# KochPJ/AutoPoseEstimation

Hardware: AMD Instinct MI355X
Metric: RGB-D frames/sec (seg+DenseFusion+2-refine), 640x480 N=1000 (higher is better)
Workload: dtype bf16x3

## Files before the change

### autoposeestimation_amd/csrc/conv_gemm.hip

```cpp
#include "s32.h"

namespace {

using namespace ape;

struct GemmArgs {
    const float* x;
    const __bf16* w;
    const float* bias;
    const float* res;
    float* y;
    ape_conv_params p;
    int M, Kp, m_tiles, n_tiles, nk;
    int out_fmt;
    int dbg;
    long plane_stride;
    int nk_per;
    long split_stride;
};

constexpr int BK = 32;

template <int NSPLIT, int BM, int BN, int WM, int WN, bool PURE, bool PP, bool SK>
__device__ __forceinline__ void conv_gemm_body(const GemmArgs& a, const int orig)
// ... 276 lines not shown
                }
            }
        }
    }
}

template <int NSPLIT, int BM, int BN, int WM, int WN, bool PURE, bool PP>
__global__ __launch_bounds__(WM * WN * 64, 2) void conv_gemm_kernel(const GemmArgs a)
{
    conv_gemm_body<NSPLIT, BM, BN, WM, WN, PURE, PP, false>(a, (int)blockIdx.x);
}

template <int NSPLIT, bool PURE>
__global__ __launch_bounds__(256, 2) void conv_gemm_splitk_kernel(const GemmArgs a)
{
    conv_gemm_body<NSPLIT, 128, 128, 2, 2, PURE, false, true>(a, (int)blockIdx.x);
}

constexpr int kMultiMax = 4;
struct GemmMultiArgs {
    GemmArgs a[kMultiMax];
    int first[kMultiMax + 1];
};
template <int NSPLIT>
__global__ __launch_bounds__(256, 2) void conv_gemm_multi_kernel(const GemmMultiArgs m)
{
    const int blk = (int)blockIdx.x;
    int pi = 0;
#pragma unroll
    for (int i = 1; i < kMultiMax; ++i) pi = blk >= m.first[i] ? i : pi;
    conv_gemm_body<NSPLIT, 128, 128, 2, 2, true, false, false>(m.a[pi], blk - m.first[pi]);
}

template <int NSPLIT, int BM, int BN, int WM, int WN, bool PP = false>
void launch(GemmArgs& a, bool pure, hipStream_t st)
{
    a.m_tiles = ape::ceil_div(a.M, BM);
    a.n_tiles = ape::ceil_div(a.p.Cout, BN);
    if (pure)
        hipLaunchKernelGGL((conv_gemm_kernel<NSPLIT, BM, BN, WM, WN, true, PP>), dim3(a.m_tiles * a.n_tiles), dim3(WM * WN * 64), 0, st, a);
    else
        hipLaunchKernelGGL((conv_gemm_kernel<NSPLIT, BM, BN, WM, WN, false, PP>), dim3(a.m_tiles * a.n_tiles), dim3(WM * WN * 64), 0, st, a);
}

template <int NSPLIT>
void launch_splitk(GemmArgs& a, bool pure, hipStream_t st)
{
    a.m_tiles = ape::ceil_div(a.M, 128);
    a.n_tiles = ape::ceil_div(a.p.Cout, 128);
    const int gy = ape::ceil_div(a.nk, a.nk_per);
    if (pure)
        hipLaunchKernelGGL((conv_gemm_splitk_kernel<NSPLIT, true>), dim3(a.m_tiles * a.n_tiles, gy), dim3(256), 0, st, a);
    else
        hipLaunchKernelGGL((conv_gemm_splitk_kernel<NSPLIT, false>), dim3(a.m_tiles * a.n_tiles, gy), dim3(256), 0, st, a);
}

__global__ void splitk_finish_kernel(const float* __restrict__ ws, int splits, long M, int Cout, const float* __restrict__ bias, int bias_bstride,
                                     int HoWo, const float* __restrict__ res, int ldr, int roff, float* __restrict__ y, int ldy, int yoff, int act,
                                     float alpha)
{
    const long n = M * Cout;
    for (long i = blockIdx.x * (long)blockDim.x + threadIdx.x; i < n; i += (long)gridDim.x * blockDim.x) {
        const long m = i / Cout;
        const int c = (int)(i - m * Cout);
        float v = ws[i];
        for (int k = 1; k < splits; ++k) v += ws[(long)k * n + i];
// ... 17 lines not shown

bool supported(const ape_conv_params& p)
{
    if (p.B < 0 || p.H < 1 || p.W < 1 || p.Cin < 32 || p.Cin % 32 || p.Cout < 1 || p.KH < 1 || p.KW < 1 || p.stride < 1 ||
        p.dil < 1 || p.pad < 0 || p.Ho < 1 || p.Wo < 1 || p.ups != 0)
        return false;
    if (p.ldx % 4 || p.xoff % 4 || p.xoff + p.Cin > p.ldx || p.yoff + p.Cout > p.ldy) return false;
    if (p.act < APE_ACT_NONE || p.act > APE_ACT_SIGMOID) return false;
    const int ho = (p.H + 2 * p.pad - p.dil * (p.KH - 1) - 1) / p.stride + 1;
    const int wo = (p.W + 2 * p.pad - p.dil * (p.KW - 1) - 1) / p.stride + 1;
    if (ho != p.Ho || wo != p.Wo) return false;
    const long M = (long)p.B * p.Ho * p.Wo;
    if (M > (1L << 30) || (long)p.B * p.H * p.W * p.ldx >= (1L << 31) || (long)p.Cout * p.KH * p.KW * p.Cin >= (1L << 31)) return false;
    return true;
}

}

extern "C" int ape_conv_gemm_supported(const ape_conv_params* params) { return params && supported(*params) ? 1 : 0; }

extern "C" int ape_conv_gemm_bf16(const float* x, const void* w_packed, const float* bias, const float* residual, float* y,
                                  const ape_conv_params* params, int nsplit, int variant, void* stream)
{
    return ape_conv_gemm_bf16_fmt(x, w_packed, bias, residual, y, APE_FMT_F32, params, nsplit, variant, stream);
}

extern "C" int ape_conv_gemm_bf16_fmt(const float* x, const void* w_packed, const float* bias, const float* residual, void* y_, int out_fmt,
                                      const ape_conv_params* params, int nsplit, int variant, void* stream)
{
    float* y = (float*)y_;
    if (out_fmt != APE_FMT_F32 && out_fmt != APE_FMT_S32) return APE_EINVAL;
    if (out_fmt == APE_FMT_S32 && params && (params->ldy % 32 || params->Cout % 4 || params->yoff % 4 || (residual && (params->ldr % 4 || params->roff % 4))))
        return APE_EINVAL;
    if (!x || !w_packed || !y || !params || (nsplit != 1 && nsplit != 3) || variant < 0 || (variant & 15) > 6) return APE_EINVAL;
    const ape_conv_params& p = *params;
    if (!supported(p)) return APE_EINVAL;
    if (residual && p.roff + p.Cout > p.ldr) return APE_EINVAL;
    const long M = (long)p.B * p.Ho * p.Wo;
    if (M == 0) return APE_OK;
    GemmArgs a;
    a.x = x; a.w = (const __bf16*)w_packed; a.bias = bias; a.res = residual; a.y = y; a.p = p;
    a.M = (int)M;
    const int K = p.KH * p.KW * p.Cin;
    a.Kp = (K + 7) / 8 * 8;
    a.nk = K / BK;
    a.plane_stride = (long)p.Cout * a.Kp;
    a.dbg = variant >> 4;
    a.out_fmt = out_fmt;
    a.nk_per = 0;
    a.split_stride = 0;
    variant &= 15;
    const bool pure = p.KH == 1 && p.KW == 1 && p.stride == 1 && p.pad == 0;
    hipStream_t st = (hipStream_t)stream;
    if (variant == 0) {
        const int waste256 = ape::ceil_div(p.Cout, 256) * 256 - p.Cout;
        const int waste192 = ape::ceil_div(p.Cout, 192) * 192 - p.Cout;
        if (p.Cout <= 64) variant = 3;
        else if (p.Cout >= 256 && waste256 * 8 <= p.Cout && K >= 256 && (long)ape::ceil_div(M, 256) * ape::ceil_div(p.Cout, 256) >= 192) variant = 1;
        else if (p.Cout >= 192 && waste192 * 8 <= p.Cout && K >= 256 && (long)ape::ceil_div(M, 256) * ape::ceil_div(p.Cout, 192) >= 192) variant = 4;
        else variant = 2;
    }
    if (variant == 1) {
        if (nsplit == 3) launch<3, 256, 256, 2, 4>(a, pure, st); else launch<1, 256, 256, 2, 4>(a, pure, st);
    } else if (variant == 2) {
        if (nsplit == 3) launch<3, 128, 128, 2, 2>(a, pure, st); else launch<1, 128, 128, 2, 2>(a, pure, st);
    } else if (variant == 3) {
        if (nsplit == 3) launch<3, 256, 64, 4, 1>(a, pure, st); else launch<1, 256, 64, 4, 1>(a, pure, st);
    } else if (variant == 4) {
        if (nsplit == 3) launch<3, 256, 192, 2, 4>(a, pure, st); else launch<1, 256, 192, 2, 4>(a, pure, st);
    } else if (variant == 5) {
        if (nsplit == 3) launch<3, 256, 256, 2, 4, true>(a, pure, st); else launch<1, 256, 256, 2, 4, true>(a, pure, st);
    } else {
        if (nsplit == 3) launch<3, 128, 192, 2, 2>(a, pure, st); else launch<1, 128, 192, 2, 2>(a, pure, st);
    }
    return ape::check_launch("ape_conv_gemm_bf16");
}

extern "C" int ape_conv_gemm_bf16_multi(int n, const float* const* x, const void* const* w_packed, const float* const* bias, float* const* y,
                                        const ape_conv_params* params, int nsplit, void* stream)
{
    if (n < 1 || n > kMultiMax || !x || !w_packed || !y || !params || (nsplit != 1 && nsplit != 3)) return APE_EINVAL;
    GemmMultiArgs m;
    int total = 0;
    for (int i = 0; i < kMultiMax; ++i) {
        m.first[i] = total;
        if (i >= n) { m.a[i] = m.a[0]; continue; }
        const ape_conv_params& p = params[i];
        if (!x[i] || !w_packed[i] || !y[i] || !supported(p) || p.KH != 1 || p.KW != 1 || p.stride != 1 || p.pad != 0) return APE_EINVAL;
        const long M = (long)p.B * p.Ho * p.Wo;
        GemmArgs& a = m.a[i];
        a.x = x[i]; a.w = (const __bf16*)w_packed[i]; a.bias = bias ? bias[i] : nullptr; a.res = nullptr; a.y = y[i]; a.p = p;
        a.M = (int)M;
        a.Kp = (p.Cin + 7) / 8 * 8;
        a.nk = p.Cin / BK;
        a.plane_stride = (long)p.Cout * a.Kp;
        a.dbg = 0;
        a.out_fmt = APE_FMT_F32;
        a.nk_per = 0;
        a.split_stride = 0;
        a.m_tiles = ape::ceil_div(a.M, 128);
        a.n_tiles = ape::ceil_div(p.Cout, 128);
        total += a.m_tiles * a.n_tiles;
// ... 54 lines not shown
```

### autoposeestimation_amd/csrc/ops.hip

```cpp
#include <map>
#include <mutex>
#include "s32.h"

namespace {

using ape::src_index;
constexpr int kThreads = 256;
constexpr int kGridCap = 8192;

__global__ void maxpool3x3s2_kernel(const float4* __restrict__ x, float4* __restrict__ y, int B, int H, int W, int C4,
                                    int Ho, int Wo)
{
    const long total = (long)B * Ho * Wo * C4;
    for (long i = blockIdx.x * (long)blockDim.x + threadIdx.x; i < total; i += (long)gridDim.x * blockDim.x) {
        const int c = i % C4;
        long t = i / C4;
        const int ox = t % Wo; t /= Wo;
        const int oy = t % Ho;
        const int b = t / Ho;
        float4 m = make_float4(-__builtin_inff(), -__builtin_inff(), -__builtin_inff(), -__builtin_inff());
#pragma unroll
        for (int ky = 0; ky < 3; ++ky) {
            const int iy = oy * 2 - 1 + ky;
            if ((unsigned)iy >= (unsigned)H) continue;
// ... 63 lines not shown
            const long row = (long)(b * H + y) * W;
#pragma unroll
            for (int a = 0; a < kPoolMaxAtoms; ++a) {
                if (a >= pl.nx) break;
                int xx = pl.xe[a];
                const int xend = pl.xe[a + 1];
                for (; xx + 4 <= xend; xx += 4) {
                    const float4 v0 = load(row + xx), v1 = load(row + xx + 1), v2 = load(row + xx + 2), v3 = load(row + xx + 3);
                    acc[a].x += v0.x; acc[a].y += v0.y; acc[a].z += v0.z; acc[a].w += v0.w;
                    acc[a].x += v1.x; acc[a].y += v1.y; acc[a].z += v1.z; acc[a].w += v1.w;
                    acc[a].x += v2.x; acc[a].y += v2.y; acc[a].z += v2.z; acc[a].w += v2.w;
                    acc[a].x += v3.x; acc[a].y += v3.y; acc[a].z += v3.z; acc[a].w += v3.w;
                }
                for (; xx < xend; ++xx) {
                    const float4 v = load(row + xx);
                    acc[a].x += v.x; acc[a].y += v.y; acc[a].z += v.z; acc[a].w += v.w;
                }
            }
        }
    }
    if (g > 0) {
#pragma unroll
        for (int a = 0; a < kPoolMaxAtoms; ++a) part[g - 1][a][lane] = acc[a];
    }
    __syncthreads();
    if (g == 0 && c < C4) {
#pragma unroll
        for (int a = 0; a < kPoolMaxAtoms; ++a) {
            if (a >= pl.nx) break;
            float4 t = acc[a];
            for (int k = 0; k < 3; ++k) { t.x += part[k][a][lane].x; t.y += part[k][a][lane].y; t.z += part[k][a][lane].z; t.w += part[k][a][lane].w; }
            atoms[(((long)b * pl.ny + ay) * pl.nx + a) * C4 + c] = t;
        }
    }
}

__global__ void avgpool_bins_kernel(const float4* __restrict__ atoms, const PoolPlan pl, int B, int H, int W, int C4, int bins_total)
{
    const long total = (long)B * bins_total * C4;
    for (long i = blockIdx.x * (long)blockDim.x + threadIdx.x; i < total; i += (long)gridDim.x * blockDim.x) {
        const int c = i % C4;
        long t = i / C4;
        int bin = t % bins_total;
        const int b = t / bins_total;
        int si = 0;
        while (bin >= pl.S[si] * pl.S[si]) { bin -= pl.S[si] * pl.S[si]; ++si; }
        const int S = pl.S[si], oy = bin / S, ox = bin - oy * S;
        float4 acc = make_float4(0.f, 0.f, 0.f, 0.f);
        for (int ay = pl.ya[si][oy]; ay < pl.yb[si][oy]; ++ay)
            for (int ax = pl.xa[si][ox]; ax < pl.xb[si][ox]; ++ax) {
                const float4 v = atoms[(((long)b * pl.ny + ay) * pl.nx + ax) * C4 + c];
                acc.x += v.x; acc.y += v.y; acc.z += v.z; acc.w += v.w;
            }
        const float inv = 1.f / (float)((pl.ye[pl.yb[si][oy]] - pl.ye[pl.ya[si][oy]]) * (pl.xe[pl.xb[si][ox]] - pl.xe[pl.xa[si][ox]]));
        reinterpret_cast<float4*>(pl.out[si])[((long)(b * S + oy) * S + ox) * C4 + c] = make_float4(acc.x * inv, acc.y * inv, acc.z * inv, acc.w * inv);
    }
}

__global__ void bilinear_kernel(const float* __restrict__ x, float* __restrict__ y, int B, int H, int W, int C4, int ldx4,
                                int Ho, int Wo, int ldy4, int yoff4, float sh, float sw, int align_corners, int accumulate)
{
    const float4* x4 = reinterpret_cast<const float4*>(x);
    float4* y4 = reinterpret_cast<float4*>(y);
    const long total = (long)B * Ho * Wo * C4;
    for (long i = blockIdx.x * (long)blockDim.x + threadIdx.x; i < total; i += (long)gridDim.x * blockDim.x) {
        const int c = i % C4;
// ... 541 lines not shown
            cuts[n++] = (o * L) / sizes[i];
            cuts[n++] = ((o + 1) * L + sizes[i] - 1) / sizes[i];
        }
    for (int i = 1; i < n; ++i)
        for (int j = i; j > 0 && cuts[j - 1] > cuts[j]; --j) { const int t = cuts[j]; cuts[j] = cuts[j - 1]; cuts[j - 1] = t; }
    int m = 0;
    for (int i = 0; i < n; ++i)
        if (m == 0 || cuts[i] != edges[m - 1]) {
            if (m > kPoolMaxAtoms) return -1;
            edges[m++] = cuts[i];
        }
    const int atoms = m - 1;
    if (atoms < 1 || atoms > kPoolMaxAtoms) return -1;
    for (int i = 0; i < nsizes; ++i)
        for (int o = 0; o < sizes[i]; ++o) {
            const int lo = (o * L) / sizes[i], hi = ((o + 1) * L + sizes[i] - 1) / sizes[i];
            int a0 = 0, a1 = 0;
            while (edges[a0] != lo) ++a0;
            while (edges[a1] != hi) ++a1;
            first[i][o] = a0;
            end[i][o] = a1;
        }
    return atoms;
}

extern "C" size_t ape_adaptive_avgpool_multi_workspace_bytes(int B, int C)
{
    return (size_t)(B < 0 ? 0 : B) * kPoolMaxAtoms * kPoolMaxAtoms * (size_t)(C < 0 ? 0 : C) * sizeof(float);
}

extern "C" int ape_adaptive_avgpool_multi_nhwc_ld(const void* x, int in_fmt, float* const* ys_host, const int* sizes_host, int nsizes, int B, int H,
                                                  int W, int C, int ldx, void* workspace, size_t workspace_bytes, void* stream)
{
    if ((in_fmt != APE_FMT_F32 && in_fmt != APE_FMT_S32) || (in_fmt == APE_FMT_S32 && (C % 32 || ldx % 32))) return APE_EINVAL;
    if (!x || !ys_host || !sizes_host || !workspace || nsizes < 1 || nsizes > kPoolMaxSizes || B < 0 || H < 1 || W < 1 || C < 4 || C % 4 ||
        ldx < C || ldx % 4)
        return APE_EINVAL;
    if (B == 0) return APE_OK;
    PoolPlan pl;
    pl.nsizes = nsizes;
    int bins_total = 0;
    for (int i = 0; i < nsizes; ++i) {
        if (sizes_host[i] < 1 || sizes_host[i] > kPoolMaxS || !ys_host[i]) return APE_EINVAL;
        pl.S[i] = sizes_host[i];
        pl.out[i] = ys_host[i];
        bins_total += sizes_host[i] * sizes_host[i];
    }
    for (int i = nsizes; i < kPoolMaxSizes; ++i) { pl.S[i] = 1 << 20; pl.out[i] = nullptr; }
    pl.ny = pool_axis_plan(H, sizes_host, nsizes, pl.ye, pl.ya, pl.yb);
    pl.nx = pool_axis_plan(W, sizes_host, nsizes, pl.xe, pl.xa, pl.xb);
    if (pl.ny < 0 || pl.nx < 0) return APE_EINVAL;
    if (workspace_bytes < (size_t)B * pl.ny * pl.nx * C * sizeof(float)) return APE_EWORKSPACE;
    hipStream_t st = (hipStream_t)stream;
    if (in_fmt == APE_FMT_S32)
        hipLaunchKernelGGL(avgpool_atoms_kernel<true>, dim3(B * pl.ny, ape::ceil_div(C / 4, 64)), dim3(256), 0, st, (const float4*)x,
                           (float4*)workspace, pl, H, W, C / 4, ldx / 4);
    else
        hipLaunchKernelGGL(avgpool_atoms_kernel<false>, dim3(B * pl.ny, ape::ceil_div(C / 4, 64)), dim3(256), 0, st, (const float4*)x,
                           (float4*)workspace, pl, H, W, C / 4, ldx / 4);
    const long total = (long)B * bins_total * (C / 4);
    hipLaunchKernelGGL(avgpool_bins_kernel, dim3(ape::grid_for(total, kThreads, kGridCap)), dim3(kThreads), 0, st, (const float4*)workspace, pl, B, H, W, C / 4,
                       bins_total);
    return ape::check_launch("ape_adaptive_avgpool_multi_nhwc_f32");
}

extern "C" int ape_bilinear_nhwc_f32(const float* x, float* y, int B, int H, int W, int C, int ldx, int Ho, int Wo, int ldy,
                                     int yoff, int align_corners, int accumulate, void* stream)
{
    if (!x || !y || B < 0 || H < 1 || W < 1 || Ho < 1 || Wo < 1 || C < 4 || C % 4 || ldx % 4 || ldy % 4 || yoff % 4 ||
        C > ldx || yoff + C > ldy)
        return APE_EINVAL;
    float sh, sw;
    if (align_corners) {
        sh = Ho > 1 ? (float)(H - 1) / (float)(Ho - 1) : 0.f;
        sw = Wo > 1 ? (float)(W - 1) / (float)(Wo - 1) : 0.f;
    } else {
        sh = (float)H / (float)Ho;
        sw = (float)W / (float)Wo;
    }
    const long total = (long)B * Ho * Wo * (C / 4);
    if (total == 0) return APE_OK;
    hipLaunchKernelGGL(bilinear_kernel, dim3(ape::grid_for(total, kThreads, kGridCap)), dim3(kThreads), 0, (hipStream_t)stream, x, y, B, H, W, C / 4,
                       ldx / 4, Ho, Wo, ldy / 4, yoff / 4, sh, sw, align_corners, accumulate);
    return ape::check_launch("ape_bilinear_nhwc_f32");
}

extern "C" int ape_gather_rows_f32(const float* x, const int64_t* index, float* y, int B, int rows_in, int n, int C, void* stream)
{
    if (!x || !index || !y || B < 0 || rows_in < 1 || n < 0 || C < 4 || C % 4) return APE_EINVAL;
    const long total = (long)B * n * (C / 4);
    if (total == 0) return APE_OK;
    hipLaunchKernelGGL(gather_rows_kernel, dim3(ape::grid_for(total, kThreads, kGridCap)), dim3(kThreads), 0, (hipStream_t)stream, (const float4*)x,
// ... 133 lines not shown
```

### autoposeestimation_amd/engine.py

```python
import contextlib
import contextvars
import ctypes
import os

import torch

from . import _lib
from ._lib import ACT_NONE, ACT_PRELU, ACT_RELU, ACT_SIGMOID, ConvParams


def _st():
    return _lib.stream_ptr()


class LaunchProfile:

    def __init__(self, only=None):
        self.records = []
        self.only = only

    def wants(self, label):
        return self.only is None or label in self.only

    def begin(self, label):
# ... 13 lines not shown
        for name, shape, flop, nbytes, e0, e1 in self.records:
            key = (name, shape) if by_shape else name
            d = out.setdefault(key, {"launches": 0, "flop": 0.0, "bytes": 0.0, "ms": 0.0})
            d["launches"] += 1
            d["flop"] += flop
            d["bytes"] += nbytes
            d["ms"] += e0.elapsed_time(e1)
        return out


def _prof_begin(label):
    prof = PROFILE
    return None if prof is None else prof.begin(label)


def _prof_end(e0, label, shape, flop, nbytes):
    if e0 is not None and PROFILE is not None:
        PROFILE.end(e0, label, shape, flop, nbytes)


def _conv_cost(conv, b, h_in, w_in, ho, wo, residual):
    flop = 2.0 * b * ho * wo * conv.cout * conv.kh * conv.kw * conv.cin_real
    nbytes = 4.0 * (b * h_in * w_in * conv.cin_real + conv.cout * conv.kh * conv.kw * conv.cin_real + b * ho * wo * conv.cout * (2 if residual else 1))
    return flop, nbytes


PROFILE = None

PRECISIONS = ("f32", "bf16x3", "bf16")
USE_HALO_KERNEL = True
USE_GEMM_KERNEL = os.environ.get("APE_USE_GEMM_KERNEL", "1") != "0"
USE_CONV_MULTI = os.environ.get("APE_USE_CONV_MULTI", "1") != "0"
GEMM_VARIANT = int(os.environ.get("APE_GEMM_VARIANT", "0"))


FMT_F32, FMT_S32 = 0, 1
USE_S32 = os.environ.get("APE_USE_S32", "1") != "0"


class S32:
    __slots__ = ("t",)

    def __init__(self, t):
        if t.dtype != torch.float32 or t.shape[-1] % 32:
            raise ValueError("S32 needs a float32 buffer with a multiple of 32 channels")
        self.t = t

    @property
    def shape(self):
        return self.t.shape

    @property
    def device(self):
        return self.t.device

    def __getitem__(self, idx):
        return S32(self.t[idx])

    def to_f32(self):
        y = torch.empty_like(self.t)
        c = self.t.shape[-1]
        _lib.call.ape_convert_s32(_lib.dptr(self.t, torch.float32), _lib.dptr(y), self.t.numel() // c, c, 0, _st())
        return y

    @staticmethod
    def from_f32(x):
# ... 104 lines not shown
        self.cin_real = cin_real
        if self.nsplit:
            if wp is None:
                raise ValueError("precision %s needs the packed bf16 planes" % precision)
            self.wp = wp
            self.variant = "conv_bf16_kernel<%d,%s>" % (self.nsplit, "128,128,2,2,64,false" if self.cout > 64 else "128,64,4,1,32,true")
        else:
            self.variant = "conv_f32_kernel<%s>" % ("128,2,2" if self.cout > 64 else "64,4,1" if self.cout > 32 else "32,4,1")
        self.stride, self.pad, self.dil, self.act, self.alpha = stride, pad, dil, act, float(alpha)
        self.splitk = bool(splitk)
        self._plans, self._ws32, self._wmx6 = {}, None, None

    def s32k(self):
        if self._ws32 is None:
            k = self.kh * self.kw * self.cin
            ws = torch.empty(self.cout * k * 2, dtype=torch.bfloat16, device=self.w.device)
            _lib.call.ape_pack_weights_s32k(_lib.dptr(self.w), _lib.dptr(ws), self.cout, k, _st())
            self._ws32 = ws
        return self._ws32

    def mx6k(self):
        if self._wmx6 is None:
            from . import mx6
            w = self.w.detach().float().cpu().numpy().reshape(self.cout, self.kh, self.kw, self.cin)
            lines = mx6.pack_lines(w.reshape(self.cout, self.kh * self.kw * (self.cin // 32), 32))
            self._wmx6 = torch.from_numpy(lines).to(self.w.device)
        return self._wmx6

    def _generic_variant(self, m):
        if self.nsplit and self.cout >= 256 and ((-(-self.cout // 256)) * 256 - self.cout) * 8 <= self.cout and m >= 65536:
            return "conv_bf16_kernel<%d,256,256,4,2,32,true>" % self.nsplit
        return self.variant

    def _gemm_variant(self, m):
        pure = "true" if (self.kh == 1 and self.kw == 1 and self.stride == 1 and self.pad == 0) else "false"
        v = GEMM_VARIANT & 15
        if v == 0:
            k = self.kh * self.kw * self.cin
            if self.cout <= 64:
                v = 3
            elif (self.cout >= 256 and ((-(-self.cout // 256)) * 256 - self.cout) * 8 <= self.cout and k >= 256
                  and -(-m // 256) * -(-self.cout // 256) >= 192):
                v = 1
            elif (self.cout >= 192 and ((-(-self.cout // 192)) * 192 - self.cout) * 8 <= self.cout and k >= 256
                  and -(-m // 256) * -(-self.cout // 192) >= 192):
                v = 4
            else:
                v = 2
        return "conv_gemm_kernel<%d,%s,%s,%s>" % (self.nsplit, {1: "256,256,2,4", 2: "128,128,2,2", 3: "256,64,4,1", 4: "256,192,2,4",
                                                               5: "256,256,2,4", 6: "128,192,2,2"}[v], pure, "true" if v == 5 else "false")

    def out_hw(self, h, w):
        ho = (h + 2 * self.pad - self.dil * (self.kh - 1) - 1) // self.stride + 1
        wo = (w + 2 * self.pad - self.dil * (self.kw - 1) - 1) // self.stride + 1
        return ho, wo

    def _make_plan(self, key):
        b, h, w, ldx, xoff, ldy, yoff, act, bias_bstride, ldr, roff, ups, splitk, in_fmt, out_fmt = key[:15]
        p = conv_params(self, b, h, w, ldx, ldy, xoff, yoff, act, bias_bstride, ldr, roff, ups)
        pref, L, m = ctypes.byref(p), _lib.lib(), b * p.Ho * p.Wo
        sk_bytes = 0
        if in_fmt == FMT_S32:
            if self.kh != 3:
                if not L.ape_conv_gemm_s32_supported(pref):
                    raise ValueError("no S32 kernel for this layer geometry (%dx%d, stride %d, Cin %d, Cout %d)" % (self.kh, self.kw, self.stride, self.cin, self.cout))
                args, entry, label = _ARGS_S32, "ape_conv_gemm_s32", gemm_s32_label(self.cout, ldr != 0)
            elif (USE_MX6 and self.cin in MX6_CIN and self.cout >= 128 and self.stride == 1 and xoff == 0 and ldx == self.cin
                  and L.ape_conv3x3_halo_mx_supported(pref)):
                args, entry, label = _ARGS_MX, "ape_conv3x3_halo_mx", halo_mx_label(self.dil)
            else:
                if not L.ape_conv3x3_halo_s32_supported(pref):
                    raise ValueError("no S32 kernel for this layer geometry (3x3, stride %d, dil %d, Cin %d, Cout %d)" % (self.stride, self.dil, self.cin, self.cout))
                args, entry, label = _ARGS_S32, "ape_conv3x3_halo_s32", halo_s32_label(self.dil)
        else:
            halo = bool(self.nsplit and USE_HALO_KERNEL and (ups or tiles16_mostly_full(h, w)) and L.ape_conv3x3_halo_supported(pref))
            gemm = bool(not halo and self.nsplit and USE_GEMM_KERNEL and L.ape_conv_gemm_supported(pref))
            if out_fmt == FMT_S32 and not gemm:
                raise ValueError("an S32 output from an fp32 input exists only on the conv_gemm kernel (Cin % 32 == 0, not a halo layer)")
            if halo:
                args, entry, label = _ARGS_BF16, "ape_conv3x3_halo_bf16", halo_label(self.nsplit, self.dil, self.cout, ups)
            elif gemm:
                sk_bytes = int(L.ape_conv_gemm_splitk_workspace_bytes(pref)) if splitk and out_fmt == FMT_F32 else 0
                args, entry = (_ARGS_SPLITK, "ape_conv_gemm_bf16_splitk") if sk_bytes else (_ARGS_GEMM, "ape_conv_gemm_bf16_fmt")
                label = self._gemm_variant(m)
            else:
                args, entry = (_ARGS_BF16, "ape_conv2d_nhwc_bf16") if self.nsplit else (_ARGS_F32, "ape_conv2d_nhwc_f32")
                label = self._generic_variant(m)
        hin, win = (h // 2, w // 2) if ups else (h, w)
        if len(self._plans) > 64:
            self._plans.clear()
        plan = self._plans[key] = (p, pref, args, getattr(_lib.call, entry), sk_bytes, label, conv_shape(self, b, p.Ho, p.Wo, ups),
                                   *_conv_cost(self, b, hin, win, p.Ho, p.Wo, ldr != 0))
        return plan

    def __call__(self, x, out=None, xoff=0, yoff=0, residual=None, roff=0, bias=None, bias_bstride=0, act=None, upsample2x=False,
                 out_fmt=FMT_F32, splitk=False):
        in_fmt = FMT_S32 if isinstance(x, S32) else FMT_F32
        if in_fmt == FMT_S32 or isinstance(residual, S32):
            if self.nsplit != 3:
                raise ValueError("S32 operands exist only in the split-bf16 ('bf16x3') precision")
            if in_fmt != FMT_S32:
                raise ValueError("S32 output / residual needs an S32 input on this path")
            if upsample2x:
                raise ValueError("no S32 kernel up-samples its input")
            x = x.t
        if upsample2x:
            can_fuse = (self.nsplit and USE_HALO_KERNEL and self.kh == 3 and self.kw == 3 and self.stride == 1 and self.pad == 1
                        and self.dil == 1 and self.cin % 32 == 0 and x.shape[3] == self.cin and xoff == 0)
            if not can_fuse:
                return self(bilinear(x, 2 * x.shape[1], 2 * x.shape[2], True), out, 0, yoff, residual, roff, bias, bias_bstride, act)
        b, h, w, ldx = x.shape
        if upsample2x:
            h, w = 2 * h, 2 * w
        ho, wo = self.out_hw(h, w)
        if out is None:
            out = torch.empty(b, ho, wo, self.cout, dtype=torch.float32, device=x.device)
        elif isinstance(out, S32):
            out = out.t
        if tuple(out.shape[:3]) != (b, ho, wo):
            raise ValueError("conv output buffer %s does not match %s" % (tuple(out.shape), (b, ho, wo)))
        res_fmt = FMT_F32
        if residual is not None:
            if isinstance(residual, S32):
                residual, res_fmt = residual.t, FMT_S32
            if tuple(residual.shape[:3]) != (b, ho, wo):
                raise ValueError("residual shape mismatch")
        bias = self.bias if bias is None else bias
        splitk = bool(splitk or (self.splitk and _POSE_STAGE.get()))
        key = (b, h, w, ldx, xoff, out.shape[3], yoff, self.act if act is None else act, bias_bstride, 0 if residual is None else residual.shape[3], roff,
               bool(upsample2x), splitk, in_fmt, out_fmt, USE_HALO_KERNEL, USE_GEMM_KERNEL, GEMM_VARIANT, USE_MX6, MX6_CIN)
        plan = self._plans.get(key) or self._make_plan(key)
        p, pref, args, fn, sk_bytes, label, shape, flop, nbytes = plan
        if p.alpha != self.alpha:
            p.alpha = self.alpha
        if args == _ARGS_MX:
            xq = torch.empty_like(x)
            _lib.call.ape_s32_to_f16m6(_lib.dptr(x, torch.float32), _lib.dptr(xq, torch.float32), b * h * w, ldx, _st())
            x = xq
        e0 = None if PROFILE is None else PROFILE.begin(label)
        xp, bp, rp, yp = _lib.dptr(x, torch.float32), _lib.dptr(bias), _lib.dptr(residual), _lib.dptr(out, torch.float32)
        if args == _ARGS_GEMM:
            fn(xp, _lib.dptr(self.wp), bp, rp, yp, out_fmt, pref, self.nsplit, GEMM_VARIANT, _st())
        elif args == _ARGS_BF16:
            fn(xp, _lib.dptr(self.wp), bp, rp, yp, pref, self.nsplit, _st())
        elif args == _ARGS_S32:
            fn(xp, _lib.dptr(self.s32k()), bp, rp, res_fmt, yp, out_fmt, pref, _st())
        elif args == _ARGS_SPLITK:
            ws = torch.empty(sk_bytes, dtype=torch.uint8, device=x.device)
            fn(xp, _lib.dptr(self.wp), bp, rp, yp, pref, self.nsplit, _lib.dptr(ws), sk_bytes, _st())
        elif args == _ARGS_MX:
            fn(xp, _lib.dptr(self.mx6k()), bp, rp, res_fmt, yp, out_fmt, pref, _st())
        else:
            fn(xp, _lib.dptr(self.w), bp, rp, yp, pref, _st())
        if e0 is not None:
            _prof_end(e0, label, shape, flop, nbytes)
        return S32(out) if out_fmt == FMT_S32 else out


def conv_seg_head(conv, x, head_w, head_b, double_softmax=True, upsample2x=False):
    b, h, w, ldx = x.shape
    if upsample2x:
        h, w = 2 * h, 2 * w
    c = head_w.shape[0]
    fusable = (conv.nsplit and USE_HALO_KERNEL and conv.cout == 64 and conv.kh == 3 and conv.kw == 3 and conv.stride == 1
               and conv.pad == 1 and conv.dil == 1 and conv.cin % 32 == 0 and ldx == conv.cin and c <= 16
               and (upsample2x or tiles16_mostly_full(h, w)))
    if not fusable:
        return seg_head(conv(x, upsample2x=upsample2x), head_w, head_b, double_softmax)
    p = conv_params(conv, b, h, w, ldx, conv.cout, ups=upsample2x)
    label = torch.empty(b, h, w, dtype=torch.uint8, device=x.device)
    score = torch.empty(b, h, w, dtype=torch.float32, device=x.device)
    hlabel = halo_label(conv.nsplit, conv.dil, conv.cout, upsample2x, head=True)
    e0 = _prof_begin(hlabel)
    _lib.call.ape_conv3x3_halo_seghead_bf16(_lib.dptr(x, torch.float32), _lib.dptr(conv.wp), _lib.dptr(conv.bias), ctypes.byref(p),
                                            conv.nsplit, _lib.dptr(head_w, torch.float32), _lib.dptr(head_b), c, _lib.dptr(label),
# ... 167 lines not shown


def gather2x2(x, code):
    b, h, w, c = x.shape
    if tuple(code.shape) != (b, h // 2, w // 2, c):
        raise ValueError("gather2x2: code %s does not pool %s" % (tuple(code.shape), tuple(x.shape)))
    y = torch.empty(b, h // 2, w // 2, c, dtype=torch.float32, device=x.device)
    _lib.call.ape_gather2x2_nhwc_f32(_lib.dptr(x, torch.float32), _lib.dptr(code, torch.uint8), _lib.dptr(y), b, h, w, c, _st())
    return y


def cross_entropy(logits, labels, n_classes=None, g=1.0, want_grad=False):
    ld = logits.shape[-1]
    c = ld if n_classes is None else int(n_classes)
    p = logits.numel() // ld
    if labels.numel() != p:
        raise ValueError("cross_entropy: %d labels for %d pixels" % (labels.numel(), p))
    out = torch.empty(2, dtype=torch.float64, device=logits.device)
    dlogits = torch.empty_like(logits) if want_grad else None
    nbytes = _lib.lib().ape_cross_entropy_workspace_bytes(p)
    ws = torch.empty(nbytes, dtype=torch.uint8, device=logits.device)
    _lib.call.ape_cross_entropy_f32(_lib.dptr(logits, torch.float32), ld, c, _lib.dptr(labels, torch.uint8), p, float(g), _lib.dptr(out),
                                    _lib.dptr(dlogits), _lib.dptr(ws), nbytes, _st())
    return out, dlogits


def adaptive_avgpool(x, s):
    b, h, w, c = x.shape
    y = torch.empty(b, s, s, c, dtype=torch.float32, device=x.device)
    _lib.call.ape_adaptive_avgpool_nhwc_f32(_lib.dptr(x, torch.float32), _lib.dptr(y), b, h, w, c, s, _st())
    return y


def adaptive_avgpool_multi(x, sizes, channels=None):
    fmt = FMT_S32 if isinstance(x, S32) else FMT_F32
    xt = x.t if fmt == FMT_S32 else x
    b, h, w, ld = xt.shape
    c = ld if channels is None else int(channels)
    sizes = list(sizes)
    ys = [torch.empty(b, s, s, c, dtype=torch.float32, device=xt.device) for s in sizes]
    ws = _workspace(_lib.lib().ape_adaptive_avgpool_multi_workspace_bytes(b, c), xt.device)
    ptrs = (ctypes.c_void_p * len(sizes))(*[y.data_ptr() for y in ys])
    szs = (ctypes.c_int * len(sizes))(*sizes)
    try:
        _lib.call.ape_adaptive_avgpool_multi_nhwc_ld(_lib.dptr(xt, torch.float32), fmt, ptrs, szs, len(sizes), b, h, w, c, ld, _lib.dptr(ws),
                                                     ws.numel() * ws.element_size(), _st())
    except _lib.ApeError as e:
        if e.code != -1:
            raise
        xf = x.to_f32() if fmt == FMT_S32 else x
        xf = xf if c == ld else xf[..., :c].contiguous()
        return {s: adaptive_avgpool(xf, s) for s in sizes}
    return dict(zip(sizes, ys))


def conv1x1_multi(convs, xs):
    convs, xs = list(convs), list(xs)
    n = len(convs)
    ok = (1 <= n <= 4 and USE_CONV_MULTI and USE_GEMM_KERNEL and not (GEMM_VARIANT & 15) and
          all(c.nsplit and c.nsplit == convs[0].nsplit and c.kh == 1 and c.kw == 1 and c.stride == 1 and c.pad == 0 and not isinstance(x, S32)
              and x.shape[3] == c.cin and x.is_contiguous() for c, x in zip(convs, xs)))
    if ok:
        outs = [torch.empty(x.shape[0], x.shape[1], x.shape[2], c.cout, dtype=torch.float32, device=x.device) for c, x in zip(convs, xs)]
        ps = (ConvParams * n)(*[conv_params(c, x.shape[0], x.shape[1], x.shape[2], x.shape[3], c.cout) for c, x in zip(convs, xs)])
        ok = all(_lib.lib().ape_conv_gemm_supported(ctypes.byref(ps[i])) for i in range(n))
    if not ok:
        return [c(x) for c, x in zip(convs, xs)]
    arr = lambda ts: (ctypes.c_void_p * n)(*[None if t is None else t.data_ptr() for t in ts])
    _lib.call.ape_conv_gemm_bf16_multi(n, arr(xs), arr([c.wp for c in convs]), arr([c.bias for c in convs]), arr(outs), ps, convs[0].nsplit, _st())
    return outs


def bilinear(x, ho, wo, align_corners, out=None, yoff=0, accumulate=False):
    b, h, w, c = x.shape
    if out is None:
        out = torch.empty(b, ho, wo, c, dtype=torch.float32, device=x.device)
    if tuple(out.shape[:3]) != (b, ho, wo):
        raise ValueError("bilinear output buffer mismatch")
# ... 594 lines not shown
```

### include/ape_hip.h

```cpp
#ifndef APE_HIP_H
#define APE_HIP_H

#include <stddef.h>
#include <stdint.h>

#ifdef __cplusplus
extern "C" {
#define APE_STATIC_ASSERT static_assert
#else
#define APE_STATIC_ASSERT _Static_assert
#endif

#define APE_OK 0
#define APE_EINVAL (-1)
#define APE_ELAUNCH (-2)
#define APE_EWORKSPACE (-3)

int ape_abi_version(void);
const char* ape_last_error(void);

int ape_knn_f32(const float* ref, const float* query, int64_t* idx,
                int batch, int dim, int ref_nb, int query_nb, int k, void* stream);

enum { APE_ACT_NONE = 0, APE_ACT_RELU = 1, APE_ACT_PRELU = 2, APE_ACT_SIGMOID = 3 };
// ... 6 lines not shown
    int32_t bias_bstride;
    int32_t ldr, roff;
    int32_t ups;
} ape_conv_params;
int ape_conv2d_nhwc_f32(const float* x, const float* w, const float* bias, const float* residual, float* y,
                        const ape_conv_params* params_host, void* stream);

long ape_packed_weights_bf16_elems(int cout, int K);
int ape_pack_weights_bf16(const float* w, void* out, int cout, int K, void* stream);
int ape_conv2d_nhwc_bf16(const float* x, const void* w_packed, const float* bias, const float* residual, float* y,
                         const ape_conv_params* params_host, int nsplit, void* stream);
int ape_conv_gemm_supported(const ape_conv_params* params_host);
int ape_conv_gemm_bf16(const float* x, const void* w_packed, const float* bias, const float* residual, float* y,
                       const ape_conv_params* params_host, int nsplit, int variant, void* stream);
enum { APE_FMT_F32 = 0, APE_FMT_S32 = 1 };
int ape_pack_weights_s32k(const float* w, void* out, int cout, int K, void* stream);
int ape_convert_s32(const void* x, void* y, long rows, int C, int to_s32, void* stream);
int ape_conv_gemm_s32_supported(const ape_conv_params* params_host);
int ape_conv3x3_halo_s32_debug(int bits);
int ape_conv_gemm_s32_debug(int bits);
int ape_conv_gemm_s32(const void* x_s32, const void* w_s32k, const float* bias, const void* residual, int res_fmt, void* y,
                      int out_fmt, const ape_conv_params* params_host, void* stream);
int ape_conv_gemm_s32_per_image(const void* x_s32, const void* w_s32k, long w_image_stride_bytes, const float* bias, void* y, int out_fmt,
                                const ape_conv_params* params_host, void* stream);
int ape_psp_fold_operands(const void* wf_s32k, const float* z1, const float* z2, const float* z3, const float* z6, void* w_out, void* x_s32,
                          int B, int h, int w, int ld, int Cin, int Cout, void* stream);
int ape_conv_gemm_bf16_fmt(const float* x, const void* w_packed, const float* bias, const float* residual, void* y, int out_fmt,
                           const ape_conv_params* params_host, int nsplit, int variant, void* stream);
int ape_conv_gemm_bf16_multi(int n, const float* const* x, const void* const* w_packed, const float* const* bias, float* const* y,
                             const ape_conv_params* params_host, int nsplit, void* stream);
size_t ape_conv_gemm_splitk_workspace_bytes(const ape_conv_params* params);
int ape_conv_gemm_bf16_splitk(const float* x, const void* w_packed, const float* bias, const float* residual, float* y,
                              const ape_conv_params* params, int nsplit, void* workspace, size_t workspace_bytes, void* stream);
int ape_adaptive_avgpool_multi_nhwc_ld(const void* x, int in_fmt, float* const* ys_host, const int* sizes_host, int nsizes, int B, int H, int W,
                                       int C, int ldx, void* workspace, size_t workspace_bytes, void* stream);
int ape_upconv3x3_gather_ex(const float* z, const float* bias, void* out, int out_fmt, int B, int h, int w, int C, int act, float alpha,
                            int fma, void* stream);
int ape_upconv3x3_gather_strip_rows(int rows);
int ape_upconv3x3_fused_supported(int h, int w, int Cin, int Cout);
int ape_upconv3x3_fused_stamps(void* device_buffer);
int ape_upconv3x3_fused_debug(int bits);
int ape_upconv3x3_fused_s32(const void* x_s32, const void* w9_s32k, const float* bias, void* out, int out_fmt, int B, int h, int w, int Cin,
                            int act, float alpha, int fma, void* stream);
int ape_upconv3x3_fused_seghead_s32(const void* x_s32, const void* w9_s32k, const float* bias, int B, int h, int w, int Cin, int act, float alpha,
                                    int fma, const float* head_w, const float* head_b, int C, uint8_t* label, float* score, int double_softmax,
                                    void* stream);
int ape_conv3x3_halo_s32_supported(const ape_conv_params* params_host);
int ape_conv3x3_halo_s32(const void* x_s32, const void* w_s32k, const float* bias, const void* residual, int res_fmt, void* y,
                         int out_fmt, const ape_conv_params* params_host, void* stream);
int ape_conv3x3_halo_mx_supported(const ape_conv_params* params_host);
int ape_conv3x3_halo_mx(const void* x_f16m6, const void* w_f16m6, const float* bias, const void* residual, int res_fmt, void* y,
                        int out_fmt, const ape_conv_params* params_host, void* stream);
int ape_conv3x3_halo_mx_debug(int bits);
int ape_s32_to_f16m6(const void* x_s32, void* y_f16m6, long pixels, int C, void* stream);
int ape_stem_conv_pool_bf16(const float* x, const float* w, const float* bias, float* y, int B, int H, int W, int nsplit,
                            void* stream);
int ape_stem_conv_pool_u8(const uint8_t* rgb, int n_frames, const int* rects, const float* w, const float* bias, float* y, int n, int Hf, int Wf,
                          int Hc, int Wc, int div255, int nsplit, void* stream);
int ape_conv3x3_halo_supported(const ape_conv_params* params_host);
int ape_conv3x3_halo_bf16(const float* x, const void* w_packed, const float* bias, const float* residual, float* y,
                          const ape_conv_params* params_host, int nsplit, void* stream);

int ape_maxpool3x3s2_nhwc_f32(const float* x, float* y, int B, int H, int W, int C, void* stream);
int ape_adaptive_avgpool_nhwc_f32(const float* x, float* y, int B, int H, int W, int C, int S, void* stream);
size_t ape_adaptive_avgpool_multi_workspace_bytes(int B, int C);
int ape_bilinear_nhwc_f32(const float* x, float* y, int B, int H, int W, int C, int ldx, int Ho, int Wo, int ldy,
// ... 421 lines not shown
```

Before: 2098.

## Add single-wave rows GEMM for small-M 1x1 convs and per-atom avgpool kernel

Adds a conv_rows_kernel that gives each 16x16 output tile to one 64-thread wave. It loads operands straight from global memory into registers with double-buffered K chunks, uses no LDS, and uses bf16x3 MFMA. It is chosen by default for pure 1x1 convs with M<=128, no residual and f32 output. The goal is more parallelism for tiny-M GEMMs, which currently launch very few large tiles. Separately, adaptive avgpool now launches one block per atom instead of one per atom row, spreading the pooling reduction over more blocks. The risks are extra redundant global loads and the cost of many tiny launches.

```diff
diff --git a/autoposeestimation_amd/csrc/conv_gemm.hip b/autoposeestimation_amd/csrc/conv_gemm.hip
--- a/autoposeestimation_amd/csrc/conv_gemm.hip
+++ b/autoposeestimation_amd/csrc/conv_gemm.hip
@@ -332,6 +332,136 @@
     conv_gemm_body<NSPLIT, 128, 128, 2, 2, true, false, false>(m.a[pi], blk - m.first[pi]);
 }
 
+constexpr int ROWS_KC = 8;
+constexpr int ROWS_MAX_M = 128;
+
+struct RowsFrag { f32x4 x0, x1; u32x4 wh, wl; };
+
+template <int NPL, int N>
+__device__ __forceinline__ void rows_load(RowsFrag (&f)[N], const float* xr, const __bf16* wr, long plane_stride, int t0)
+{
+#pragma unroll
+    for (int i = 0; i < N; ++i) {
+        const int k = (t0 + i) * BK;
+        f[i].x0 = *reinterpret_cast<const f32x4*>(xr + k);
+        f[i].x1 = *reinterpret_cast<const f32x4*>(xr + k + 4);
+        f[i].wh = *reinterpret_cast<const u32x4*>(wr + k);
+        if (NPL == 2) f[i].wl = *reinterpret_cast<const u32x4*>(wr + plane_stride + k);
+    }
+}
+
+template <int NPL, int N>
+__device__ __forceinline__ void rows_mfma(const RowsFrag (&f)[N], f32x4& acc)
+{
+#pragma unroll
+    for (int i = 0; i < N; ++i) {
+        bf16x8 ah, al;
+        split8(f[i].x0, f[i].x1, ah, al);
+        const bf16x8 bh = __builtin_bit_cast(bf16x8, f[i].wh);
+        if (NPL == 2) {
+            const bf16x8 bl = __builtin_bit_cast(bf16x8, f[i].wl);
+            acc = __builtin_amdgcn_mfma_f32_16x16x32_bf16(bh, al, acc, 0, 0, 0);
+            acc = __builtin_amdgcn_mfma_f32_16x16x32_bf16(bl, ah, acc, 0, 0, 0);
+        }
+        acc = __builtin_amdgcn_mfma_f32_16x16x32_bf16(bh, ah, acc, 0, 0, 0);
+    }
+}
+
+template <int NSPLIT>
+__global__ __launch_bounds__(64) void conv_rows_kernel(const GemmArgs a)
+{
+    constexpr int NPL = NSPLIT == 3 ? 2 : 1;
+    constexpr int KC = ROWS_KC;
+    const ape_conv_params& p = a.p;
+    const int lane = threadIdx.x;
+    const int frow = lane & 15, fc = lane >> 4;
+    const int xcd = (int)blockIdx.x % 8, seq = (int)blockIdx.x / 8;
+    const int n0 = ((seq / a.m_tiles) * 8 + xcd) * 16;
+    const int mb = (seq % a.m_tiles) * 16;
+    if (n0 >= p.Cout) return;
+
+    const int m = mb + frow;
+    const bool mok = m < a.M;
+    const int mc = mok ? m : a.M - 1;
+    const int nw = n0 + frow < p.Cout ? n0 + frow : p.Cout - 1;
+    const float* const xr = a.x + (size_t)mc * p.ldx + p.xoff + fc * 8;
+    const __bf16* const wr = a.w + (size_t)nw * a.Kp + fc * 8;
+
+    f32x4 acc = {0.f, 0.f, 0.f, 0.f};
+    const int nk = a.nk;
+    int t = 0;
+    if (nk >= KC) {
+        RowsFrag fa[KC], fb[KC];
+        rows_load<NPL, KC>(fa, xr, wr, a.plane_stride, 0);
+#pragma unroll 1
+        for (;;) {
+            const bool more_b = t + 2 * KC <= nk;
+            if (more_b) rows_load<NPL, KC>(fb, xr, wr, a.plane_stride, t + KC);
+            rows_mfma<NPL, KC>(fa, acc);
+            t += KC;
+            if (!more_b) break;
+            const bool more_a = t + 2 * KC <= nk;
+            if (more_a) rows_load<NPL, KC>(fa, xr, wr, a.plane_stride, t + KC);
+            rows_mfma<NPL, KC>(fb, acc);
+            t += KC;
+            if (!more_a) break;
+        }
+    }
+    if (nk - t >= 4) {
+        RowsFrag f[4];
+        rows_load<NPL, 4>(f, xr, wr, a.plane_stride, t);
+        rows_mfma<NPL, 4>(f, acc);
+        t += 4;
+    }
+    if (nk - t >= 2) {
+        RowsFrag f[2];
+        rows_load<NPL, 2>(f, xr, wr, a.plane_stride, t);
+        rows_mfma<NPL, 2>(f, acc);
+        t += 2;
+    }
+    if (nk - t >= 1) {
+        RowsFrag f[1];
+        rows_load<NPL, 1>(f, xr, wr, a.plane_stride, t);
+        rows_mfma<NPL, 1>(f, acc);
+    }
+
+    const int n = n0 + fc * 4;
+    if (!mok || n >= p.Cout) return;
+    const bool vec_ok = (p.ldy % 4 == 0) && (p.yoff % 4 == 0);
+    const ape::ActFast af = ape::act_fast_make(p.act, p.alpha);
+    const bool sigm = p.act == APE_ACT_SIGMOID;
+    const float* brow = (a.bias && p.bias_bstride) ? a.bias + (size_t)(m / (p.Ho * p.Wo)) * p.bias_bstride : nullptr;
+    float vv[4] = {acc[0], acc[1], acc[2], acc[3]};
+    const int nvalid = min(4, p.Cout - n);
+    if (vec_ok && nvalid == 4) {
+        if (brow) { vv[0] += brow[n]; vv[1] += brow[n + 1]; vv[2] += brow[n + 2]; vv[3] += brow[n + 3]; }
+        else if (a.bias) { vv[0] += a.bias[n]; vv[1] += a.bias[n + 1]; vv[2] += a.bias[n + 2]; vv[3] += a.bias[n + 3]; }
+        const float4 o4 = sigm ? make_float4(activate(vv[0], p.act, p.alpha), activate(vv[1], p.act, p.alpha), activate(vv[2], p.act, p.alpha),
+                                             activate(vv[3], p.act, p.alpha))
+                               : make_float4(ape::act_fast(vv[0], af), ape::act_fast(vv[1], af), ape::act_fast(vv[2], af), ape::act_fast(vv[3], af));
+        *reinterpret_cast<float4*>(a.y + (size_t)m * p.ldy + p.yoff + n) = o4;
+    } else {
+        for (int k = 0; k < nvalid; ++k) {
+            float tv = vv[k];
+            if (a.bias) tv += (brow ? brow : a.bias)[n + k];
+            a.y[(size_t)m * p.ldy + p.yoff + n + k] = activate(tv, p.act, p.alpha);
+        }
+    }
+}
+
+bool rows_takes(const GemmArgs& a, bool pure)
+{
+    return pure && !a.res && a.out_fmt == APE_FMT_F32 && ((long)ape::ceil_div(a.p.Cout, 16) + 7) * ape::ceil_div(a.M, 16) < (1L << 31);
+}
+
+template <int NSPLIT>
+void launch_rows(GemmArgs& a, hipStream_t st)
+{
+    a.m_tiles = ape::ceil_div(a.M, 16);
+    a.n_tiles = ape::ceil_div(a.p.Cout, 16);
+    hipLaunchKernelGGL((conv_rows_kernel<NSPLIT>), dim3(ape::ceil_div(a.n_tiles, 8) * 8 * a.m_tiles), dim3(64), 0, st, a);
+}
+
 template <int NSPLIT, int BM, int BN, int WM, int WN, bool PP = false>
 void launch(GemmArgs& a, bool pure, hipStream_t st)
 {
@@ -415,7 +545,7 @@
     if (out_fmt != APE_FMT_F32 && out_fmt != APE_FMT_S32) return APE_EINVAL;
     if (out_fmt == APE_FMT_S32 && params && (params->ldy % 32 || params->Cout % 4 || params->yoff % 4 || (residual && (params->ldr % 4 || params->roff % 4))))
         return APE_EINVAL;
-    if (!x || !w_packed || !y || !params || (nsplit != 1 && nsplit != 3) || variant < 0 || (variant & 15) > 6) return APE_EINVAL;
+    if (!x || !w_packed || !y || !params || (nsplit != 1 && nsplit != 3) || variant < 0 || (variant & 15) > 7) return APE_EINVAL;
     const ape_conv_params& p = *params;
     if (!supported(p)) return APE_EINVAL;
     if (residual && p.roff + p.Cout > p.ldr) return APE_EINVAL;
@@ -435,10 +565,12 @@
     variant &= 15;
     const bool pure = p.KH == 1 && p.KW == 1 && p.stride == 1 && p.pad == 0;
     hipStream_t st = (hipStream_t)stream;
+    if (variant == 7 && !rows_takes(a, pure)) return APE_EINVAL;
     if (variant == 0) {
         const int waste256 = ape::ceil_div(p.Cout, 256) * 256 - p.Cout;
         const int waste192 = ape::ceil_div(p.Cout, 192) * 192 - p.Cout;
-        if (p.Cout <= 64) variant = 3;
+        if (M <= ROWS_MAX_M && !(a.dbg & 16) && rows_takes(a, pure)) variant = 7;
+        else if (p.Cout <= 64) variant = 3;
         else if (p.Cout >= 256 && waste256 * 8 <= p.Cout && K >= 256 && (long)ape::ceil_div(M, 256) * ape::ceil_div(p.Cout, 256) >= 192) variant = 1;
         else if (p.Cout >= 192 && waste192 * 8 <= p.Cout && K >= 256 && (long)ape::ceil_div(M, 256) * ape::ceil_div(p.Cout, 192) >= 192) variant = 4;
         else variant = 2;
@@ -451,6 +583,8 @@
         if (nsplit == 3) launch<3, 256, 64, 4, 1>(a, pure, st); else launch<1, 256, 64, 4, 1>(a, pure, st);
     } else if (variant == 4) {
         if (nsplit == 3) launch<3, 256, 192, 2, 4>(a, pure, st); else launch<1, 256, 192, 2, 4>(a, pure, st);
+    } else if (variant == 7) {
+        if (nsplit == 3) launch_rows<3>(a, st); else launch_rows<1>(a, st);
     } else if (variant == 5) {
         if (nsplit == 3) launch<3, 256, 256, 2, 4, true>(a, pure, st); else launch<1, 256, 256, 2, 4, true>(a, pure, st);
     } else {
diff --git a/autoposeestimation_amd/csrc/ops.hip b/autoposeestimation_amd/csrc/ops.hip
--- a/autoposeestimation_amd/csrc/ops.hip
+++ b/autoposeestimation_amd/csrc/ops.hip
@@ -119,6 +119,43 @@
             for (int k = 0; k < 3; ++k) { t.x += part[k][a][lane].x; t.y += part[k][a][lane].y; t.z += part[k][a][lane].z; t.w += part[k][a][lane].w; }
             atoms[(((long)b * pl.ny + ay) * pl.nx + a) * C4 + c] = t;
         }
+    }
+}
+
+template <bool S32IN>
+__global__ __launch_bounds__(256) void avgpool_atom_kernel(const float4* __restrict__ x, float4* __restrict__ atoms, const PoolPlan pl,
+                                                           int H, int W, int C4, int ld4)
+{
+    __shared__ float4 part[3][64];
+    const int lane = threadIdx.x & 63, g = threadIdx.x >> 6;
+    const int ax = blockIdx.x % pl.nx, ay = (blockIdx.x / pl.nx) % pl.ny, b = blockIdx.x / (pl.nx * pl.ny);
+    const int c = blockIdx.y * 64 + lane;
+    float4 acc = make_float4(0.f, 0.f, 0.f, 0.f);
+    if (c < C4) {
+        auto load = [&](long pix) { return S32IN ? ape::s32_load4(x, pix, ld4, c) : x[pix * ld4 + c]; };
+        auto add = [&](const float4 v) { acc.x += v.x; acc.y += v.y; acc.z += v.z; acc.w += v.w; };
+        const int x0 = pl.xe[ax], xend = pl.xe[ax + 1];
+        for (int y = pl.ye[ay] + g; y < pl.ye[ay + 1]; y += 4) {
+            const long row = (long)(b * H + y) * W;
+            int xx = x0;
+            for (; xx + 8 <= xend; xx += 8) {
+                const float4 v0 = load(row + xx), v1 = load(row + xx + 1), v2 = load(row + xx + 2), v3 = load(row + xx + 3);
+                const float4 v4 = load(row + xx + 4), v5 = load(row + xx + 5), v6 = load(row + xx + 6), v7 = load(row + xx + 7);
+                add(v0); add(v1); add(v2); add(v3); add(v4); add(v5); add(v6); add(v7);
+            }
+            for (; xx + 4 <= xend; xx += 4) {
+                const float4 v0 = load(row + xx), v1 = load(row + xx + 1), v2 = load(row + xx + 2), v3 = load(row + xx + 3);
+                add(v0); add(v1); add(v2); add(v3);
+            }
+            for (; xx < xend; ++xx) add(load(row + xx));
+        }
+    }
+    if (g > 0) part[g - 1][lane] = acc;
+    __syncthreads();
+    if (g == 0 && c < C4) {
+        float4 t = acc;
+        for (int k = 0; k < 3; ++k) { t.x += part[k][lane].x; t.y += part[k][lane].y; t.z += part[k][lane].z; t.w += part[k][lane].w; }
+        atoms[(((long)b * pl.ny + ay) * pl.nx + ax) * C4 + c] = t;
     }
 }
 
@@ -726,6 +763,8 @@
 extern "C" int ape_adaptive_avgpool_multi_nhwc_ld(const void* x, int in_fmt, float* const* ys_host, const int* sizes_host, int nsizes, int B, int H,
                                                   int W, int C, int ldx, void* workspace, size_t workspace_bytes, void* stream)
 {
+    const bool atom_rows = in_fmt >= 0 && (in_fmt & APE_POOL_ATOM_ROWS);
+    if (in_fmt >= 0) in_fmt &= ~APE_POOL_ATOM_ROWS;
     if ((in_fmt != APE_FMT_F32 && in_fmt != APE_FMT_S32) || (in_fmt == APE_FMT_S32 && (C % 32 || ldx % 32))) return APE_EINVAL;
     if (!x || !ys_host || !sizes_host || !workspace || nsizes < 1 || nsizes > kPoolMaxSizes || B < 0 || H < 1 || W < 1 || C < 4 || C % 4 ||
         ldx < C || ldx % 4)
@@ -746,12 +785,15 @@
     if (pl.ny < 0 || pl.nx < 0) return APE_EINVAL;
     if (workspace_bytes < (size_t)B * pl.ny * pl.nx * C * sizeof(float)) return APE_EWORKSPACE;
     hipStream_t st = (hipStream_t)stream;
-    if (in_fmt == APE_FMT_S32)
-        hipLaunchKernelGGL(avgpool_atoms_kernel<true>, dim3(B * pl.ny, ape::ceil_div(C / 4, 64)), dim3(256), 0, st, (const float4*)x,
-                           (float4*)workspace, pl, H, W, C / 4, ldx / 4);
-    else
-        hipLaunchKernelGGL(avgpool_atoms_kernel<false>, dim3(B * pl.ny, ape::ceil_div(C / 4, 64)), dim3(256), 0, st, (const float4*)x,
-                           (float4*)workspace, pl, H, W, C / 4, ldx / 4);
+    if ((long)B * pl.ny * pl.nx >= (1L << 31)) return APE_EINVAL;
+    const dim3 grid(atom_rows ? B * pl.ny : B * pl.ny * pl.nx, ape::ceil_div(C / 4, 64));
+    if (in_fmt == APE_FMT_S32) {
+        if (atom_rows) hipLaunchKernelGGL(avgpool_atoms_kernel<true>, grid, dim3(256), 0, st, (const float4*)x, (float4*)workspace, pl, H, W, C / 4, ldx / 4);
+        else hipLaunchKernelGGL(avgpool_atom_kernel<true>, grid, dim3(256), 0, st, (const float4*)x, (float4*)workspace, pl, H, W, C / 4, ldx / 4);
+    } else {
+        if (atom_rows) hipLaunchKernelGGL(avgpool_atoms_kernel<false>, grid, dim3(256), 0, st, (const float4*)x, (float4*)workspace, pl, H, W, C / 4, ldx / 4);
+        else hipLaunchKernelGGL(avgpool_atom_kernel<false>, grid, dim3(256), 0, st, (const float4*)x, (float4*)workspace, pl, H, W, C / 4, ldx / 4);
+    }
     const long total = (long)B * bins_total * (C / 4);
     hipLaunchKernelGGL(avgpool_bins_kernel, dim3(ape::grid_for(total, kThreads, kGridCap)), dim3(kThreads), 0, st, (const float4*)workspace, pl, B, H, W, C / 4,
                        bins_total);
diff --git a/autoposeestimation_amd/engine.py b/autoposeestimation_amd/engine.py
--- a/autoposeestimation_amd/engine.py
+++ b/autoposeestimation_amd/engine.py
@@ -69,6 +69,8 @@
 USE_GEMM_KERNEL = os.environ.get("APE_USE_GEMM_KERNEL", "1") != "0"
 USE_CONV_MULTI = os.environ.get("APE_USE_CONV_MULTI", "1") != "0"
 GEMM_VARIANT = int(os.environ.get("APE_GEMM_VARIANT", "0"))
+USE_GEMM_ROWS = os.environ.get("APE_USE_GEMM_ROWS", "1") != "0"
+GEMM_ROWS_MAX_M = 128
 
 
 FMT_F32, FMT_S32 = 0, 1
@@ -239,12 +241,15 @@
             return "conv_bf16_kernel<%d,256,256,4,2,32,true>" % self.nsplit
         return self.variant
 
-    def _gemm_variant(self, m):
+    def _gemm_variant(self, m, residual=False, out_fmt=FMT_F32):
         pure = "true" if (self.kh == 1 and self.kw == 1 and self.stride == 1 and self.pad == 0) else "false"
         v = GEMM_VARIANT & 15
         if v == 0:
             k = self.kh * self.kw * self.cin
-            if self.cout <= 64:
+            if (m <= GEMM_ROWS_MAX_M and USE_GEMM_ROWS and not (GEMM_VARIANT & 0x100) and pure == "true" and not residual
+                    and out_fmt == FMT_F32):
+                v = 7
+            elif self.cout <= 64:
                 v = 3
             elif (self.cout >= 256 and ((-(-self.cout // 256)) * 256 - self.cout) * 8 <= self.cout and k >= 256
                   and -(-m // 256) * -(-self.cout // 256) >= 192):
@@ -254,6 +259,8 @@
                 v = 4
             else:
                 v = 2
+        if v == 7:
+            return "conv_rows_kernel<%d>" % self.nsplit
         return "conv_gemm_kernel<%d,%s,%s,%s>" % (self.nsplit, {1: "256,256,2,4", 2: "128,128,2,2", 3: "256,64,4,1", 4: "256,192,2,4",
                                                                5: "256,256,2,4", 6: "128,192,2,2"}[v], pure, "true" if v == 5 else "false")
 
@@ -289,7 +296,7 @@
             elif gemm:
                 sk_bytes = int(L.ape_conv_gemm_splitk_workspace_bytes(pref)) if splitk and out_fmt == FMT_F32 else 0
                 args, entry = (_ARGS_SPLITK, "ape_conv_gemm_bf16_splitk") if sk_bytes else (_ARGS_GEMM, "ape_conv_gemm_bf16_fmt")
-                label = self._gemm_variant(m)
+                label = self._gemm_variant(m, ldr != 0, out_fmt)
             else:
                 args, entry = (_ARGS_BF16, "ape_conv2d_nhwc_bf16") if self.nsplit else (_ARGS_F32, "ape_conv2d_nhwc_f32")
                 label = self._generic_variant(m)
@@ -335,7 +342,7 @@
         bias = self.bias if bias is None else bias
         splitk = bool(splitk or (self.splitk and _POSE_STAGE.get()))
         key = (b, h, w, ldx, xoff, out.shape[3], yoff, self.act if act is None else act, bias_bstride, 0 if residual is None else residual.shape[3], roff,
-               bool(upsample2x), splitk, in_fmt, out_fmt, USE_HALO_KERNEL, USE_GEMM_KERNEL, GEMM_VARIANT, USE_MX6, MX6_CIN)
+               bool(upsample2x), splitk, in_fmt, out_fmt, USE_HALO_KERNEL, USE_GEMM_KERNEL, GEMM_VARIANT, USE_MX6, MX6_CIN, USE_GEMM_ROWS)
         plan = self._plans.get(key) or self._make_plan(key)
         p, pref, args, fn, sk_bytes, label, shape, flop, nbytes = plan
         if p.alpha != self.alpha:
@@ -347,7 +354,7 @@
         e0 = None if PROFILE is None else PROFILE.begin(label)
         xp, bp, rp, yp = _lib.dptr(x, torch.float32), _lib.dptr(bias), _lib.dptr(residual), _lib.dptr(out, torch.float32)
         if args == _ARGS_GEMM:
-            fn(xp, _lib.dptr(self.wp), bp, rp, yp, out_fmt, pref, self.nsplit, GEMM_VARIANT, _st())
+            fn(xp, _lib.dptr(self.wp), bp, rp, yp, out_fmt, pref, self.nsplit, GEMM_VARIANT if USE_GEMM_ROWS else GEMM_VARIANT | 0x100, _st())
         elif args == _ARGS_BF16:
             fn(xp, _lib.dptr(self.wp), bp, rp, yp, pref, self.nsplit, _st())
         elif args == _ARGS_S32:
@@ -581,6 +588,9 @@
     return y
 
 
+POOL_ATOM_ROWS = False
+
+
 def adaptive_avgpool_multi(x, sizes, channels=None):
     fmt = FMT_S32 if isinstance(x, S32) else FMT_F32
     xt = x.t if fmt == FMT_S32 else x
@@ -592,7 +602,7 @@
     ptrs = (ctypes.c_void_p * len(sizes))(*[y.data_ptr() for y in ys])
     szs = (ctypes.c_int * len(sizes))(*sizes)
     try:
-        _lib.call.ape_adaptive_avgpool_multi_nhwc_ld(_lib.dptr(xt, torch.float32), fmt, ptrs, szs, len(sizes), b, h, w, c, ld, _lib.dptr(ws),
+        _lib.call.ape_adaptive_avgpool_multi_nhwc_ld(_lib.dptr(xt, torch.float32), fmt | (0x100 if POOL_ATOM_ROWS else 0), ptrs, szs, len(sizes), b, h, w, c, ld, _lib.dptr(ws),
                                                      ws.numel() * ws.element_size(), _st())
     except _lib.ApeError as e:
         if e.code != -1:
diff --git a/include/ape_hip.h b/include/ape_hip.h
--- a/include/ape_hip.h
+++ b/include/ape_hip.h
@@ -62,6 +62,7 @@
 size_t ape_conv_gemm_splitk_workspace_bytes(const ape_conv_params* params);
 int ape_conv_gemm_bf16_splitk(const float* x, const void* w_packed, const float* bias, const float* residual, float* y,
                               const ape_conv_params* params, int nsplit, void* workspace, size_t workspace_bytes, void* stream);
+enum { APE_POOL_ATOM_ROWS = 0x100 };
 int ape_adaptive_avgpool_multi_nhwc_ld(const void* x, int in_fmt, float* const* ys_host, const int* sizes_host, int nsizes, int B, int H, int W,
                                        int C, int ldx, void* workspace, size_t workspace_bytes, void* stream);
 int ape_upconv3x3_gather_ex(const float* z, const float* bias, void* out, int out_fmt, int B, int h, int w, int C, int act, float alpha,
```

Measured after the change: 2127 (median of 6 runs). +1.4%, better.
